# spartan-array/spartan

Hardware: AMD Instinct MI355X
Metric: spartan.dot TFLOP/s (+ map/reduce HBM GB/s) (higher is better)
Workload: dtype f32

## Files before the change

### spartan_amd/csrc/gemm_split.hpp

```cpp
#pragma once

typedef __bf16 gs_bf16x8 __attribute__((ext_vector_type(8)));
typedef __bf16 gs_bf16x4 __attribute__((ext_vector_type(4)));

namespace {

constexpr int GS_BK = 16;
constexpr int GS_RB = GS_BK * 2;
constexpr int GS_WN = 4;
constexpr unsigned GS_WIN_LO = (127u - 40u) << 23;
constexpr unsigned GS_WIN_HI = (127u + 40u) << 23;
constexpr size_t GS_IMAGE_CAP = (size_t)2 << 30;
constexpr size_t GS_WS_HEAD = 512;

template <int WN>
struct GsCfg {
  static constexpr int BM = 256, BN = 64 * WN, NW = 2 * WN, THREADS = 64 * NW;
  static constexpr int A_BYTES = BM * GS_RB, B_BYTES = BN * GS_RB;
  static constexpr int STAGE_BYTES = 3 * A_BYTES + 3 * B_BYTES;
  static constexpr int SMEM_BYTES = 2 * STAGE_BYTES;
  static constexpr int APW = A_BYTES / 1024 / NW, BPW = B_BYTES / 1024 / NW;
  static constexpr int NPIECES = 3 * APW + 3 * BPW;
  static constexpr int SLOTS = SP_CUS * (WN == 4 ? 1 : 2);
  static_assert(APW >= 1 && BPW >= 1 && APW * NW * 1024 == A_BYTES && BPW * NW * 1024 == B_BYTES, "tile / waves mismatch");
  static_assert(NPIECES * 4 <= 48, "one piece after every fourth MFMA");
};

template <int V>
struct GsInt {
  static constexpr int value = V;
};

__device__ __forceinline__ bool gs_outside(float v) {
  const unsigned b = __float_as_uint(v) & 0x7fffffffu;
  return b != 0u && (b < GS_WIN_LO || b >= GS_WIN_HI);
}

__device__ __forceinline__ void gs_cut(float v, __bf16& h, __bf16& m, __bf16& l) {
  h = (__bf16)v;
  const float r1 = v - (float)h;
  m = (__bf16)r1;
  l = (__bf16)(r1 - (float)m);
}

__device__ __forceinline__ void gs_raise(bool bad, unsigned* flag) {
  if (__any(bad) && (threadIdx.x & 63) == 0) atomicOr(flag, 1u);
}

__global__ __launch_bounds__(256) void sp_gemm_cut_rows_kernel(const float* __restrict__ A, int64_t lda, int M, int K,
                                                               __bf16* __restrict__ Ah, int64_t img,
                                                               unsigned* __restrict__ flag) {
  const int q = threadIdx.x & 7, row = blockIdx.x * 32 + (threadIdx.x >> 3);
  const int kpad = (K + GS_BK - 1) / GS_BK * GS_BK;
  bool bad = false;
  if (row < M) {
    const float* __restrict__ a = A + (int64_t)row * lda;
#pragma unroll
    for (int it = 0; it < 8; ++it) {
      const int k = blockIdx.y * 256 + it * 32 + 4 * q;
      if (k >= kpad) break;
      f32x4 v = {0.f, 0.f, 0.f, 0.f};
      if (k + 4 <= K) {
        v = *(const f32x4*)(a + k);
      } else {
#pragma unroll
        for (int e = 0; e < 4; ++e)
          if (k + e < K) v[e] = a[k + e];
      }
      gs_bf16x4 h, m, l;
#pragma unroll
      for (int e = 0; e < 4; ++e) {
        bad |= gs_outside(v[e]);
        __bf16 hh, mm, ll;
        gs_cut(v[e], hh, mm, ll);
        h[e] = hh;
        m[e] = mm;
        l[e] = ll;
      }
      const int64_t at = ((int64_t)(k >> 4) * M + row) * GS_BK + (k & 15);
      *(gs_bf16x4*)(Ah + at) = h;
      *(gs_bf16x4*)(Ah + img + at) = m;
      *(gs_bf16x4*)(Ah + 2 * img + at) = l;
    }
  }
  gs_raise(bad, flag);
}

__global__ __launch_bounds__(256) void sp_gemm_cut_cols_kernel(const float* __restrict__ B, int64_t ldb, int N, int K,
                                                               __bf16* __restrict__ Bh, int64_t img,
                                                               unsigned* __restrict__ flag) {
  __shared__ __attribute__((aligned(16))) __bf16 s[3][256 * GS_BK];
  const int n0 = blockIdx.x * 256, col = n0 + threadIdx.x, k0 = blockIdx.y * GS_BK;
  float v[GS_BK];
#pragma unroll
  for (int e = 0; e < GS_BK; ++e) v[e] = (col < N && k0 + e < K) ? B[(int64_t)(k0 + e) * ldb + col] : 0.f;
  bool bad = false;
  gs_bf16x8 h[2], m[2], l[2];
#pragma unroll
  for (int e = 0; e < GS_BK; ++e) {
    bad |= gs_outside(v[e]);
    __bf16 hh, mm, ll;
    gs_cut(v[e], hh, mm, ll);
    h[e >> 3][e & 7] = hh;
    m[e >> 3][e & 7] = mm;
    l[e >> 3][e & 7] = ll;
  }
#pragma unroll
  for (int c = 0; c < 2; ++c) {
    *(gs_bf16x8*)(&s[0][threadIdx.x * GS_BK + 8 * c]) = h[c];
    *(gs_bf16x8*)(&s[1][threadIdx.x * GS_BK + 8 * c]) = m[c];
    *(gs_bf16x8*)(&s[2][threadIdx.x * GS_BK + 8 * c]) = l[c];
  }
  __syncthreads();
  const int64_t base = ((int64_t)blockIdx.y * N + n0) * GS_BK;
#pragma unroll
  for (int p = 0; p < 3; ++p)
#pragma unroll
    for (int c = 0; c < 2; ++c) {
      const int at = (c * 256 + threadIdx.x) * 8;
      if (n0 + at / GS_BK < N) *(gs_bf16x8*)(Bh + p * img + base + at) = *(const gs_bf16x8*)(&s[p][at]);
    }
  gs_raise(bad, flag);
}

template <int WN>
__global__ __launch_bounds__(GsCfg<WN>::THREADS, 2) void sp_gemm_glds_kernel_bf16x3(
    const char* __restrict__ Ah, int64_t a_img, const char* __restrict__ Bh, int64_t b_img, float* __restrict__ C,
    int64_t ldc, int M, int N, int KT, int accumulate, int tiles_m, int tiles_n, int64_t a_slab, int64_t b_slab,
    const unsigned* __restrict__ flag_a, const unsigned* __restrict__ flag_b) {
  using G = GsCfg<WN>;
  constexpr int APW = G::APW, BPW = G::BPW, NPIECES = G::NPIECES;
  extern __shared__ __attribute__((aligned(16))) char gs_smem[];
  if ((*flag_a | *flag_b) != 0u) return;
  int tm, tn;
  sp_gemm_tile_of_block(blockIdx.x, gridDim.x, tiles_m, tiles_n, tm, tn);
  const int m0 = tm * G::BM, n0 = tn * G::BN;
  const int tid = threadIdx.x, lane = tid & 63;
  const int wid = __builtin_amdgcn_readfirstlane(tid >> 6);
  const int wm = wid / WN, wn = wid % WN;
  const int l31 = lane & 31, lh = lane >> 5;

  unsigned a_off[APW], b_off[BPW];
#pragma unroll
  for (int j = 0; j < APW; ++j) {
    const int slot = (wid * APW + j) * 64 + lane;
    int row = slot >> 1;
    const int q = (slot & 1) ^ ((row >> 4) & 1);
    if (m0 + row > M - 1) row = M - 1 - m0;
    a_off[j] = (unsigned)(row * GS_RB + q * 16);
  }
#pragma unroll
  for (int j = 0; j < BPW; ++j) {
    const int slot = (wid * BPW + j) * 64 + lane;
    int row = slot >> 1;
    const int q = (slot & 1) ^ ((row >> 4) & 1);
    if (n0 + row > N - 1) row = N - 1 - n0;
    b_off[j] = (unsigned)(row * GS_RB + q * 16);
  }
  const char* __restrict__ Ablk = Ah + (int64_t)m0 * GS_RB;
  const char* __restrict__ Bblk = Bh + (int64_t)n0 * GS_RB;
  const unsigned s_base = SP_LDS_ADDR(gs_smem);

#define GS_PIECE(i)                                                                                    \
  do {                                                                                                 \
    if ((i) < 3 * APW) {                                                                               \
      const int p_ = (i) / APW, j_ = (i) % APW;                                                        \
      SP_GLDS_S(Ablk + p_ * a_img + ka_, a_off[j_], st_ + p_ * G::A_BYTES + (wid * APW + j_) * 1024);  \
    } else {                                                                                           \
      const int p_ = ((i) - 3 * APW) / BPW, j_ = ((i) - 3 * APW) % BPW;                                \
      SP_GLDS_S(Bblk + p_ * b_img + kb_, b_off[j_],                                                    \
                st_ + 3 * G::A_BYTES + p_ * G::B_BYTES + (wid * BPW + j_) * 1024);                     \
    }                                                                                                  \
  } while (0)

  f32x16 acc[4][2];
#pragma unroll
  for (int i = 0; i < 4; ++i)
#pragma unroll
    for (int j = 0; j < 2; ++j)
#pragma unroll
      for (int r = 0; r < 16; ++r) acc[i][j][r] = 0.f;

  const int fslot = (lh ^ ((l31 >> 4) & 1)) * 16;
  const int a_frag = (wm * 128 + l31) * GS_RB + fslot;
  const int b_frag = 3 * G::A_BYTES + (wn * 64 + l31) * GS_RB + fslot;
  const unsigned a_rd[2] = {s_base + (unsigned)a_frag, s_base + (unsigned)(G::STAGE_BYTES + a_frag)};
  const unsigned b_rd[2] = {s_base + (unsigned)b_frag, s_base + (unsigned)(G::STAGE_BYTES + b_frag)};

  gs_bf16x8 am[4], al[4], bm[2], bl[2], ah[2][4], bh[2][2];
#define GS_READ_A(dst, s_, p_, i_) \
  asm volatile("ds_read_b128 %0, %1 offset:%2" : "+v"(dst) : "v"(a_rd[s_]), "n"((p_) * G::A_BYTES + (i_) * 32 * GS_RB) : "memory")
#define GS_READ_B(dst, s_, p_, j_) \
  asm volatile("ds_read_b128 %0, %1 offset:%2" : "+v"(dst) : "v"(b_rd[s_]), "n"((p_) * G::B_BYTES + (j_) * 32 * GS_RB) : "memory")
#define GS_READS_DONE(s_)                                                                                             \
  do {                                                                                                                \
    asm volatile("s_waitcnt lgkmcnt(0)"                                                                               \
                 : "+v"(al[0]), "+v"(al[1]), "+v"(al[2]), "+v"(al[3]), "+v"(am[0]), "+v"(am[1]), "+v"(am[2]),          \
                   "+v"(am[3]), "+v"(bl[0]), "+v"(bl[1]), "+v"(bm[0]), "+v"(bm[1])                                     \
                 :: "memory");                                                                                        \
    asm volatile("" : "+v"(ah[s_][0]), "+v"(ah[s_][1]), "+v"(ah[s_][2]), "+v"(ah[s_][3]), "+v"(bh[s_][0]),             \
                      "+v"(bh[s_][1]) :: "memory");                                                                   \
  } while (0)

  auto ktile = [&](auto par_, const bool rd, const bool ld, int t) __attribute__((always_inline)) {
    constexpr int CUR = decltype(par_)::value, NXT = CUR ^ 1;
    const int64_t ka_ = (int64_t)(t + 2) * a_slab, kb_ = (int64_t)(t + 2) * b_slab;
    const unsigned st_ = s_base + (unsigned)CUR * G::STAGE_BYTES;
#pragma unroll
    for (int idx = 0; idx < 48; ++idx) {
      const int term = idx >> 3, i = (idx & 7) >> 1, j = idx & 1;
      const gs_bf16x8 a = term == 0 ? al[i] : (term == 2 || term == 3) ? am[i] : ah[CUR][i];
      const gs_bf16x8 b = term == 1 ? bl[j] : (term == 2 || term == 4) ? bm[j] : bh[CUR][j];
      acc[i][j] = __builtin_amdgcn_mfma_f32_32x32x16_bf16(a, b, acc[i][j], 0, 0, 0);
      __builtin_amdgcn_sched_barrier(0);
      if (rd) {
        const int q = idx & 7, r = q < 3 ? q : q - 1;
        if (term == 0 && q != 3 && q != 7) {
          if (r < 4) GS_READ_A(ah[NXT][r & 3], NXT, 0, r & 3);
          else GS_READ_B(bh[NXT][r & 1], NXT, 0, r & 1);
        }
        if (term == 1 && q != 3 && r < 4) GS_READ_A(al[r & 3], NXT, 2, r & 3);
        if (term == 2 && q < 2) GS_READ_B(bl[q & 1], NXT, 2, q & 1);
        if (term == 4 && q < 4) GS_READ_A(am[q & 3], NXT, 1, q & 3);
        if (term == 5 && q < 2) GS_READ_B(bm[q & 1], NXT, 1, q & 1);
      }
      if (ld && idx % 4 == 3 && idx / 4 < NPIECES) GS_PIECE(idx / 4);
      __builtin_amdgcn_sched_barrier(0);
    }
    if (ld) SP_GLDS_LANDED();
    if (rd) GS_READS_DONE(NXT);
    __syncthreads();
    __builtin_amdgcn_sched_barrier(0);
  };
  GsInt<0> even;
  GsInt<1> odd;

  {
    const int64_t ka_ = 0, kb_ = 0;
    const unsigned st_ = s_base;
#pragma unroll
    for (int i = 0; i < NPIECES; ++i) GS_PIECE(i);
  }
  SP_GLDS_LANDED();
  __syncthreads();
  if (KT > 1) {
    const int64_t ka_ = a_slab, kb_ = b_slab;
    const unsigned st_ = s_base + G::STAGE_BYTES;
#pragma unroll
    for (int i = 0; i < NPIECES; ++i) GS_PIECE(i);
  }
#pragma unroll
  for (int i = 0; i < 4; ++i) {
    ah[0][i] = ah[1][i] = am[i] = al[i] = gs_bf16x8{};
    GS_READ_A(ah[0][i], 0, 0, i);
    GS_READ_A(am[i], 0, 1, i);
    GS_READ_A(al[i], 0, 2, i);
  }
#pragma unroll
  for (int j = 0; j < 2; ++j) {
    bh[0][j] = bh[1][j] = bm[j] = bl[j] = gs_bf16x8{};
    GS_READ_B(bh[0][j], 0, 0, j);
    GS_READ_B(bm[j], 0, 1, j);
    GS_READ_B(bl[j], 0, 2, j);
  }
  SP_GLDS_LANDED();
  GS_READS_DONE(0);
  __syncthreads();

  int t = 0;
  for (; t + 1 < KT; t += 2) {
    ktile(even, true, t + 2 < KT, t);
    ktile(odd, t + 2 < KT, t + 3 < KT, t + 1);
  }
  if (t < KT) ktile(even, false, false, t);
#undef GS_READ_A
#undef GS_READ_B
#undef GS_READS_DONE
#undef GS_PIECE

#pragma unroll
  for (int i = 0; i < 4; ++i) {
#pragma unroll
    for (int j = 0; j < 2; ++j) {
      const int col = n0 + wn * 64 + j * 32 + l31;
#pragma unroll
      for (int r = 0; r < 16; ++r) {
        const int row = m0 + wm * 128 + i * 32 + (r & 3) + 8 * (r >> 2) + 4 * lh;
        if (row < M && col < N) {
          float* p = C + (int64_t)row * ldc + col;
          float v = acc[i][j][r];
          if (accumulate) v += *p;
          *p = v;
        }
      }
    }
  }
}

template <typename Cfg, int BM, int BN, int WM, int WN, int WGS>
__global__ __launch_bounds__(Cfg::THREADS, WGS) void sp_gemm_f32_gated_kernel(
    const float* __restrict__ A, int64_t lda, const float* __restrict__ B, int64_t ldb, float* __restrict__ C,
    int64_t ldc, int M, int N, int K, int accumulate, int tiles_m, int tiles_n, const unsigned* __restrict__ flag_a,
    const unsigned* __restrict__ flag_b) {
  if ((*flag_a | *flag_b) == 0u) return;
  sp_gemm_glds_body<Cfg, BM, BN, WM, WN>(A, lda, B, ldb, C, ldc, M, N, K, accumulate, tiles_m, tiles_n);
}

#define GS_CUT_BYTES_PER_S 3.0e12
#define GS_ISSUED_FLOPS 1.1e15
static bool sp_gemm_bf16_plan(int64_t M, int64_t N, int64_t K) {
  static int mode = -2;
  if (mode == -2) {
    const char* e = getenv("SP_GEMM_SPLIT");
    mode = e ? atoi(e) : 1;
  }
  using G = GsCfg<GS_WN>;
  if (mode == 0 || K < 16 || N % 4 != 0 || N < 4 || M < 1 || M > 2147483647LL || N > 2147483647LL || K > 2147483647LL)
    return false;
  const int64_t tb = ((M + 255) / 256) * ((N + 127) / 128);
  if (tb < 2 * SP_CUS || tb >= 2147483647LL) return false;
  double dp_cost;
  if (sp_gemm_dp_choice(M, N, &dp_cost) != 6 || sp_sk_plan(M, N, K)) return false;
  const int64_t KT = (K + GS_BK - 1) / GS_BK;
  if ((double)KT * 3.0 * GS_RB * ((double)M + (double)N) > (double)GS_IMAGE_CAP) return false;
  const double fp32_s = dp_cost * 128.0 * 128.0 * (double)K * 2.0 / (157.3e12 * 0.95 / SP_CUS);
  const int64_t tiles = ((M + G::BM - 1) / G::BM) * ((N + G::BN - 1) / G::BN);
  const int64_t rounds = (tiles + G::SLOTS - 1) / G::SLOTS;
  const double main_s = (double)rounds * G::SLOTS * (6.0 * 2.0 * G::BM * G::BN * (double)K) / GS_ISSUED_FLOPS;
  const double cut_s = 10.0 * ((double)M + (double)N) * (double)K / GS_CUT_BYTES_PER_S;
  return (main_s + cut_s + 20e-6) < 0.92 * fp32_s;
}

static size_t sp_gemm_bf16_ws_bytes(int64_t M, int64_t N, int64_t K) {
  return GS_WS_HEAD + (size_t)((K + GS_BK - 1) / GS_BK) * 3 * GS_RB * (size_t)(M + N);
}

constexpr size_t GS_IMG_HEAD = 256;

static size_t sp_gemm_bf16_image_bytes(int64_t rows, int64_t K) {
  return GS_IMG_HEAD + (size_t)((K + GS_BK - 1) / GS_BK) * 3 * GS_RB * (size_t)rows;
}

static long long gs_cut_launches = 0;

static void sp_gemm_bf16_cut(int side, const float* X, int64_t ld, int64_t rows, int64_t K, char* img, unsigned* flag,
                             hipStream_t st) {
  const int64_t KT = (K + GS_BK - 1) / GS_BK;
  const int64_t img_stride = KT * rows * GS_RB;
  __atomic_add_fetch(&gs_cut_launches, 1, __ATOMIC_RELAXED);
  if (side == 0)
    hipLaunchKernelGGL(sp_gemm_cut_rows_kernel, dim3((unsigned)((rows + 31) / 32), (unsigned)((K + 255) / 256)), dim3(256), 0,
                       st, X, ld, (int)rows, (int)K, (__bf16*)img, img_stride / 2, flag);
  else
    hipLaunchKernelGGL(sp_gemm_cut_cols_kernel, dim3((unsigned)((rows + 255) / 256), (unsigned)KT), dim3(256), 0, st, X, ld,
                       (int)rows, (int)K, (__bf16*)img, img_stride / 2, flag);
}

static int sp_gemm_bf16_launch(const float* A, int64_t lda, const char* imgA, int64_t a_rows, int64_t a_row0,
                               const float* B, int64_t ldb, const char* imgB, int64_t b_rows, int64_t b_row0, float* C,
                               int64_t ldc, int64_t M, int64_t N, int64_t K, int acc, void* ws, hipStream_t st) {
  using G = GsCfg<GS_WN>;
  const int64_t KT = (K + GS_BK - 1) / GS_BK;
  const int64_t tiles_m = (M + G::BM - 1) / G::BM, tiles_n = (N + G::BN - 1) / G::BN;
  auto kern = sp_gemm_glds_kernel_bf16x3<GS_WN>;
  using FCfg = GldsCfg<256, 128, 2, 2>;
  auto gated = sp_gemm_f32_gated_kernel<FCfg, 256, 128, 2, 2, 2>;
  static bool attr_set = false;
  if (!attr_set) {
    SP_HIP(hipFuncSetAttribute((const void*)kern, hipFuncAttributeMaxDynamicSharedMemorySize, G::SMEM_BYTES));
    SP_HIP(hipFuncSetAttribute((const void*)gated, hipFuncAttributeMaxDynamicSharedMemorySize, FCfg::LDS_BYTES));
    attr_set = true;
  }
  char* base = (char*)(((uintptr_t)ws + 255) & ~(uintptr_t)255);
  char* next = base + GS_IMG_HEAD;
  if (!imgA || !imgB) SP_HIP(hipMemsetAsync(base, 0, GS_IMG_HEAD, st));
  const unsigned* flag_a = (const unsigned*)(imgA ? imgA : base);
  const unsigned* flag_b = (const unsigned*)(imgB ? imgB : base);
  const char *Ah, *Bh;
  if (imgA) {
    Ah = imgA + GS_IMG_HEAD + a_row0 * GS_RB;
  } else {
    a_rows = M;
    sp_gemm_bf16_cut(0, A, lda, M, K, next, (unsigned*)base, st);
    Ah = next;
    next += 3 * KT * M * GS_RB;
  }
  if (imgB) {
    Bh = imgB + GS_IMG_HEAD + b_row0 * GS_RB;
  } else {
    b_rows = N;
    sp_gemm_bf16_cut(1, B, ldb, N, K, next, (unsigned*)base, st);
    Bh = next;
  }
  hipLaunchKernelGGL(kern, dim3((unsigned)(tiles_m * tiles_n)), dim3(G::THREADS), G::SMEM_BYTES, st, Ah,
                     KT * a_rows * GS_RB, Bh, KT * b_rows * GS_RB, C, ldc, (int)M, (int)N, (int)KT, acc, (int)tiles_m,
                     (int)tiles_n, a_rows * GS_RB, b_rows * GS_RB, flag_a, flag_b);
  const int64_t ftm = (M + 255) / 256, ftn = (N + 127) / 128;
  hipLaunchKernelGGL(gated, dim3((unsigned)(ftm * ftn)), dim3(FCfg::THREADS), FCfg::LDS_BYTES, st, A, lda, B, ldb, C, ldc,
                     (int)M, (int)N, (int)K, acc, (int)ftm, (int)ftn, flag_a, flag_b);
  SP_CHECK_LAUNCH();
  return 0;
}

}
```

Measured before the change: 262.4.

## Restructure bf16x3 split GEMM into 4-wave 256x256 tiles with 16x16x32 MFMA

Reworks the bf16x3 split-precision GEMM kernel from 8 waves with 32x32x16 MFMAs and 6 product terms to 4 waves, each owning a 128x128 sub-tile of 16x16x32 MFMAs with accumulators pinned in AGPRs. The three-term products are packed so lanes in the upper half read different precision images, which cuts the MFMA issue count per k-tile. LDS reads and global-to-LDS pieces are reinterleaved via a compile-time unrolled schedule. The loads are now unconditional, clamped to the last tile, which removes branches but issues redundant loads at the tail. Occupancy drops to one block per CU with heavy register use.

```diff
diff --git a/spartan_amd/csrc/gemm_split.hpp b/spartan_amd/csrc/gemm_split.hpp
--- a/spartan_amd/csrc/gemm_split.hpp
+++ b/spartan_amd/csrc/gemm_split.hpp
@@ -1,4 +1,5 @@
 #pragma once
+#include <utility>
 
 typedef __bf16 gs_bf16x8 __attribute__((ext_vector_type(8)));
 typedef __bf16 gs_bf16x4 __attribute__((ext_vector_type(4)));
@@ -7,29 +8,34 @@
 
 constexpr int GS_BK = 16;
 constexpr int GS_RB = GS_BK * 2;
-constexpr int GS_WN = 4;
 constexpr unsigned GS_WIN_LO = (127u - 40u) << 23;
 constexpr unsigned GS_WIN_HI = (127u + 40u) << 23;
 constexpr size_t GS_IMAGE_CAP = (size_t)2 << 30;
 constexpr size_t GS_WS_HEAD = 512;
 
-template <int WN>
 struct GsCfg {
-  static constexpr int BM = 256, BN = 64 * WN, NW = 2 * WN, THREADS = 64 * NW;
+  static constexpr int BM = 256, BN = 256, NW = 4, THREADS = 64 * NW;
   static constexpr int A_BYTES = BM * GS_RB, B_BYTES = BN * GS_RB;
   static constexpr int STAGE_BYTES = 3 * A_BYTES + 3 * B_BYTES;
   static constexpr int SMEM_BYTES = 2 * STAGE_BYTES;
   static constexpr int APW = A_BYTES / 1024 / NW, BPW = B_BYTES / 1024 / NW;
   static constexpr int NPIECES = 3 * APW + 3 * BPW;
-  static constexpr int SLOTS = SP_CUS * (WN == 4 ? 1 : 2);
+  static constexpr int SLOTS = SP_CUS;
+  static constexpr int NMFMA = 3 * 8 * 8;
   static_assert(APW >= 1 && BPW >= 1 && APW * NW * 1024 == A_BYTES && BPW * NW * 1024 == B_BYTES, "tile / waves mismatch");
-  static_assert(NPIECES * 4 <= 48, "one piece after every fourth MFMA");
+  static_assert(NPIECES * 8 <= NMFMA / 2, "one piece after every eighth MFMA of the first half");
+  static_assert(STAGE_BYTES + 7 * 16 * GS_RB < 65536, "stage and block go into a ds_read's 16-bit offset");
 };
 
 template <int V>
 struct GsInt {
   static constexpr int value = V;
 };
+
+template <int... I, typename F>
+__device__ __forceinline__ void gs_unrolled(std::integer_sequence<int, I...>, F&& f) {
+  (f(GsInt<I>{}), ...);
+}
 
 __device__ __forceinline__ bool gs_outside(float v) {
   const unsigned b = __float_as_uint(v) & 0x7fffffffu;
@@ -123,12 +129,11 @@
   gs_raise(bad, flag);
 }
 
-template <int WN>
-__global__ __launch_bounds__(GsCfg<WN>::THREADS, 2) void sp_gemm_glds_kernel_bf16x3(
+__global__ __launch_bounds__(GsCfg::THREADS, 1) void sp_gemm_glds_kernel_bf16x3(
     const char* __restrict__ Ah, int64_t a_img, const char* __restrict__ Bh, int64_t b_img, float* __restrict__ C,
     int64_t ldc, int M, int N, int KT, int accumulate, int tiles_m, int tiles_n, int64_t a_slab, int64_t b_slab,
     const unsigned* __restrict__ flag_a, const unsigned* __restrict__ flag_b) {
-  using G = GsCfg<WN>;
+  using G = GsCfg;
   constexpr int APW = G::APW, BPW = G::BPW, NPIECES = G::NPIECES;
   extern __shared__ __attribute__((aligned(16))) char gs_smem[];
   if ((*flag_a | *flag_b) != 0u) return;
@@ -137,8 +142,8 @@
   const int m0 = tm * G::BM, n0 = tn * G::BN;
   const int tid = threadIdx.x, lane = tid & 63;
   const int wid = __builtin_amdgcn_readfirstlane(tid >> 6);
-  const int wm = wid / WN, wn = wid % WN;
-  const int l31 = lane & 31, lh = lane >> 5;
+  const int wm = wid >> 1, wn = wid & 1;
+  const int l15 = lane & 15, lq = lane >> 4;
 
   unsigned a_off[APW], b_off[BPW];
 #pragma unroll
@@ -173,62 +178,71 @@
     }                                                                                                  \
   } while (0)
 
-  f32x16 acc[4][2];
-#pragma unroll
-  for (int i = 0; i < 4; ++i)
-#pragma unroll
-    for (int j = 0; j < 2; ++j)
-#pragma unroll
-      for (int r = 0; r < 16; ++r) acc[i][j][r] = 0.f;
-
-  const int fslot = (lh ^ ((l31 >> 4) & 1)) * 16;
-  const int a_frag = (wm * 128 + l31) * GS_RB + fslot;
-  const int b_frag = 3 * G::A_BYTES + (wn * 64 + l31) * GS_RB + fslot;
-  const unsigned a_rd[2] = {s_base + (unsigned)a_frag, s_base + (unsigned)(G::STAGE_BYTES + a_frag)};
-  const unsigned b_rd[2] = {s_base + (unsigned)b_frag, s_base + (unsigned)(G::STAGE_BYTES + b_frag)};
-
-  gs_bf16x8 am[4], al[4], bm[2], bl[2], ah[2][4], bh[2][2];
-#define GS_READ_A(dst, s_, p_, i_) \
-  asm volatile("ds_read_b128 %0, %1 offset:%2" : "+v"(dst) : "v"(a_rd[s_]), "n"((p_) * G::A_BYTES + (i_) * 32 * GS_RB) : "memory")
-#define GS_READ_B(dst, s_, p_, j_) \
-  asm volatile("ds_read_b128 %0, %1 offset:%2" : "+v"(dst) : "v"(b_rd[s_]), "n"((p_) * G::B_BYTES + (j_) * 32 * GS_RB) : "memory")
-#define GS_READS_DONE(s_)                                                                                             \
-  do {                                                                                                                \
-    asm volatile("s_waitcnt lgkmcnt(0)"                                                                               \
-                 : "+v"(al[0]), "+v"(al[1]), "+v"(al[2]), "+v"(al[3]), "+v"(am[0]), "+v"(am[1]), "+v"(am[2]),          \
-                   "+v"(am[3]), "+v"(bl[0]), "+v"(bl[1]), "+v"(bm[0]), "+v"(bm[1])                                     \
-                 :: "memory");                                                                                        \
-    asm volatile("" : "+v"(ah[s_][0]), "+v"(ah[s_][1]), "+v"(ah[s_][2]), "+v"(ah[s_][3]), "+v"(bh[s_][0]),             \
-                      "+v"(bh[s_][1]) :: "memory");                                                                   \
+  f32x4 acc[8][8];
+#define GS_MFMA(c, a, b) asm volatile("v_mfma_f32_16x16x32_bf16 %0, %1, %2, %0" : "+a"(c) : "v"(a), "v"(b))
+#define GS_ACC_ZEROED(c) asm volatile("" : "+a"(c))
+#define GS_ACC_DONE(x)                                                                                              \
+  asm volatile("s_nop 7\n\ts_nop 7\n\ts_nop 3"                                                                      \
+               : "+a"(x[0]), "+a"(x[1]), "+a"(x[2]), "+a"(x[3]), "+a"(x[4]), "+a"(x[5]), "+a"(x[6]), "+a"(x[7]))
+#pragma unroll
+  for (int i = 0; i < 8; ++i)
+#pragma unroll
+    for (int j = 0; j < 8; ++j) {
+      acc[i][j] = f32x4{0.f, 0.f, 0.f, 0.f};
+      GS_ACC_ZEROED(acc[i][j]);
+    }
+
+  const int up = lane >> 5;
+  unsigned a_rd[2][2], b_rd[3][2];
+#pragma unroll
+  for (int par = 0; par < 2; ++par) {
+    const unsigned a_row = s_base + (unsigned)((wm * 128 + l15) * GS_RB + (((lq & 1) ^ par) * 16));
+    const unsigned b_row = s_base + (unsigned)(3 * G::A_BYTES + (wn * 128 + l15) * GS_RB + (((lq & 1) ^ par) * 16));
+    a_rd[0][par] = a_row + (unsigned)((up ? 0 : 2) * G::A_BYTES);
+    a_rd[1][par] = a_row + (unsigned)((up ? 0 : 1) * G::A_BYTES);
+    b_rd[0][par] = b_row + (unsigned)((up ? 2 : 0) * G::B_BYTES);
+    b_rd[1][par] = b_row + (unsigned)((up ? 1 : 0) * G::B_BYTES);
+    b_rd[2][par] = b_row + (unsigned)((up ? 0 : 1) * G::B_BYTES);
+  }
+
+  gs_bf16x8 a_lh[8], b_hl[8], b_hm[8], a_mh[2][8], b_mh[2][8];
+#define GS_READ_A(dst, s_, v_, blk_)                                       \
+  asm volatile("ds_read_b128 %0, %1 offset:%2" : "+v"(dst) : "v"(a_rd[v_][(blk_) & 1]), \
+               "n"((s_) * G::STAGE_BYTES + (blk_) * 16 * GS_RB) : "memory")
+#define GS_READ_B(dst, s_, v_, blk_)                                       \
+  asm volatile("ds_read_b128 %0, %1 offset:%2" : "+v"(dst) : "v"(b_rd[v_][(blk_) & 1]), \
+               "n"((s_) * G::STAGE_BYTES + (blk_) * 16 * GS_RB) : "memory")
+#define GS_TIE8(x) "+v"(x[0]), "+v"(x[1]), "+v"(x[2]), "+v"(x[3]), "+v"(x[4]), "+v"(x[5]), "+v"(x[6]), "+v"(x[7])
+#define GS_READS_DONE(s_)                                                                              \
+  do {                                                                                                 \
+    asm volatile("s_waitcnt lgkmcnt(0)" : GS_TIE8(a_lh), GS_TIE8(b_hl), GS_TIE8(b_hm) :: "memory");    \
+    asm volatile("" : GS_TIE8(a_mh[s_]), GS_TIE8(b_mh[s_]) :: "memory");                               \
   } while (0)
 
-  auto ktile = [&](auto par_, const bool rd, const bool ld, int t) __attribute__((always_inline)) {
+  auto ktile = [&](auto par_, int t) __attribute__((always_inline)) {
     constexpr int CUR = decltype(par_)::value, NXT = CUR ^ 1;
-    const int64_t ka_ = (int64_t)(t + 2) * a_slab, kb_ = (int64_t)(t + 2) * b_slab;
+    const int tl = t + 2 < KT ? t + 2 : KT - 1;
+    const int64_t ka_ = (int64_t)tl * a_slab, kb_ = (int64_t)tl * b_slab;
     const unsigned st_ = s_base + (unsigned)CUR * G::STAGE_BYTES;
-#pragma unroll
-    for (int idx = 0; idx < 48; ++idx) {
-      const int term = idx >> 3, i = (idx & 7) >> 1, j = idx & 1;
-      const gs_bf16x8 a = term == 0 ? al[i] : (term == 2 || term == 3) ? am[i] : ah[CUR][i];
-      const gs_bf16x8 b = term == 1 ? bl[j] : (term == 2 || term == 4) ? bm[j] : bh[CUR][j];
-      acc[i][j] = __builtin_amdgcn_mfma_f32_32x32x16_bf16(a, b, acc[i][j], 0, 0, 0);
+    gs_unrolled(std::make_integer_sequence<int, G::NMFMA>{}, [&](auto idx_) __attribute__((always_inline)) {
+      constexpr int idx = decltype(idx_)::value, term = idx >> 6, i = (idx >> 3) & 7, j = idx & 7;
+      const gs_bf16x8 a = term == 0 ? a_lh[i] : a_mh[CUR][i];
+      const gs_bf16x8 b = term == 0 ? b_hl[j] : term == 1 ? b_hm[j] : b_mh[CUR][j];
+      GS_MFMA(acc[i][j], a, b);
       __builtin_amdgcn_sched_barrier(0);
-      if (rd) {
-        const int q = idx & 7, r = q < 3 ? q : q - 1;
-        if (term == 0 && q != 3 && q != 7) {
-          if (r < 4) GS_READ_A(ah[NXT][r & 3], NXT, 0, r & 3);
-          else GS_READ_B(bh[NXT][r & 1], NXT, 0, r & 1);
-        }
-        if (term == 1 && q != 3 && r < 4) GS_READ_A(al[r & 3], NXT, 2, r & 3);
-        if (term == 2 && q < 2) GS_READ_B(bl[q & 1], NXT, 2, q & 1);
-        if (term == 4 && q < 4) GS_READ_A(am[q & 3], NXT, 1, q & 3);
-        if (term == 5 && q < 2) GS_READ_B(bm[q & 1], NXT, 1, q & 1);
+      if constexpr ((idx & 3) == 0) {
+        constexpr int q = (idx & 63) >> 2, blk = q & 7;
+        if constexpr (term == 0 && q < 8) GS_READ_A(a_mh[NXT][blk], NXT, 1, blk);
+        if constexpr (term == 0 && q >= 8) GS_READ_B(b_mh[NXT][blk], NXT, 2, blk);
+        if constexpr (term == 1 && q < 8) GS_READ_A(a_lh[blk], NXT, 0, blk);
+        if constexpr (term == 1 && q >= 8) GS_READ_B(b_hl[blk], NXT, 0, blk);
+        if constexpr (term == 2 && q < 8) GS_READ_B(b_hm[blk], NXT, 1, blk);
       }
-      if (ld && idx % 4 == 3 && idx / 4 < NPIECES) GS_PIECE(idx / 4);
+      if constexpr (idx % 8 == 7 && idx / 8 < NPIECES) GS_PIECE(idx / 8);
       __builtin_amdgcn_sched_barrier(0);
-    }
-    if (ld) SP_GLDS_LANDED();
-    if (rd) GS_READS_DONE(NXT);
+    });
+    SP_GLDS_LANDED();
+    GS_READS_DONE(NXT);
     __syncthreads();
     __builtin_amdgcn_sched_barrier(0);
   };
@@ -243,25 +257,20 @@
   }
   SP_GLDS_LANDED();
   __syncthreads();
-  if (KT > 1) {
-    const int64_t ka_ = a_slab, kb_ = b_slab;
+  {
+    const int64_t ka_ = KT > 1 ? a_slab : 0, kb_ = KT > 1 ? b_slab : 0;
     const unsigned st_ = s_base + G::STAGE_BYTES;
 #pragma unroll
     for (int i = 0; i < NPIECES; ++i) GS_PIECE(i);
   }
 #pragma unroll
-  for (int i = 0; i < 4; ++i) {
-    ah[0][i] = ah[1][i] = am[i] = al[i] = gs_bf16x8{};
-    GS_READ_A(ah[0][i], 0, 0, i);
-    GS_READ_A(am[i], 0, 1, i);
-    GS_READ_A(al[i], 0, 2, i);
-  }
-#pragma unroll
-  for (int j = 0; j < 2; ++j) {
-    bh[0][j] = bh[1][j] = bm[j] = bl[j] = gs_bf16x8{};
-    GS_READ_B(bh[0][j], 0, 0, j);
-    GS_READ_B(bm[j], 0, 1, j);
-    GS_READ_B(bl[j], 0, 2, j);
+  for (int blk = 0; blk < 8; ++blk) {
+    a_lh[blk] = a_mh[0][blk] = a_mh[1][blk] = b_hl[blk] = b_hm[blk] = b_mh[0][blk] = b_mh[1][blk] = gs_bf16x8{};
+    GS_READ_A(a_lh[blk], 0, 0, blk);
+    GS_READ_A(a_mh[0][blk], 0, 1, blk);
+    GS_READ_B(b_hl[blk], 0, 0, blk);
+    GS_READ_B(b_hm[blk], 0, 1, blk);
+    GS_READ_B(b_mh[0][blk], 0, 2, blk);
   }
   SP_GLDS_LANDED();
   GS_READS_DONE(0);
@@ -269,28 +278,37 @@
 
   int t = 0;
   for (; t + 1 < KT; t += 2) {
-    ktile(even, true, t + 2 < KT, t);
-    ktile(odd, t + 2 < KT, t + 3 < KT, t + 1);
-  }
-  if (t < KT) ktile(even, false, false, t);
+    ktile(even, t);
+    ktile(odd, t + 1);
+  }
+  if (t < KT) ktile(even, t);
+  GS_ACC_DONE(acc[7]);
+#undef GS_MFMA
+#undef GS_ACC_ZEROED
+#undef GS_ACC_DONE
 #undef GS_READ_A
 #undef GS_READ_B
 #undef GS_READS_DONE
+#undef GS_TIE8
 #undef GS_PIECE
 
 #pragma unroll
-  for (int i = 0; i < 4; ++i) {
-#pragma unroll
-    for (int j = 0; j < 2; ++j) {
-      const int col = n0 + wn * 64 + j * 32 + l31;
-#pragma unroll
-      for (int r = 0; r < 16; ++r) {
-        const int row = m0 + wm * 128 + i * 32 + (r & 3) + 8 * (r >> 2) + 4 * lh;
-        if (row < M && col < N) {
-          float* p = C + (int64_t)row * ldc + col;
-          float v = acc[i][j][r];
-          if (accumulate) v += *p;
-          *p = v;
+  for (int i = 0; i < 8; ++i) {
+#pragma unroll
+    for (int jp = 0; jp < 8; jp += 2) {
+#pragma unroll
+      for (int r = 0; r < 4; ++r) {
+        const int row = m0 + wm * 128 + i * 16 + 4 * lq + r;
+#pragma unroll
+        for (int j = jp; j < jp + 2; ++j) {
+          const int col = n0 + wn * 128 + j * 16 + l15;
+          if (row < M && col < N) {
+            float* p = C + (int64_t)row * ldc + col;
+            float v;
+            asm volatile("v_accvgpr_read_b32 %0, %1" : "=v"(v) : "a"(acc[i][j][r]));
+            if (accumulate) v += *p;
+            *p = v;
+          }
         }
       }
     }
@@ -314,7 +332,7 @@
     const char* e = getenv("SP_GEMM_SPLIT");
     mode = e ? atoi(e) : 1;
   }
-  using G = GsCfg<GS_WN>;
+  using G = GsCfg;
   if (mode == 0 || K < 16 || N % 4 != 0 || N < 4 || M < 1 || M > 2147483647LL || N > 2147483647LL || K > 2147483647LL)
     return false;
   const int64_t tb = ((M + 255) / 256) * ((N + 127) / 128);
@@ -359,10 +377,10 @@
 static int sp_gemm_bf16_launch(const float* A, int64_t lda, const char* imgA, int64_t a_rows, int64_t a_row0,
                                const float* B, int64_t ldb, const char* imgB, int64_t b_rows, int64_t b_row0, float* C,
                                int64_t ldc, int64_t M, int64_t N, int64_t K, int acc, void* ws, hipStream_t st) {
-  using G = GsCfg<GS_WN>;
+  using G = GsCfg;
   const int64_t KT = (K + GS_BK - 1) / GS_BK;
   const int64_t tiles_m = (M + G::BM - 1) / G::BM, tiles_n = (N + G::BN - 1) / G::BN;
-  auto kern = sp_gemm_glds_kernel_bf16x3<GS_WN>;
+  auto kern = sp_gemm_glds_kernel_bf16x3;
   using FCfg = GldsCfg<256, 128, 2, 2>;
   auto gated = sp_gemm_f32_gated_kernel<FCfg, 256, 128, 2, 2, 2>;
   static bool attr_set = false;
```

After: 285.2, median of 6. +8.7%, better.
